# Seasandwpy/viso

Measured on AMD Instinct MI355X. Metric: stereo frames/sec at 1242x375 grey, 1/2/4/8 GPUs; pose RMSE vs reference, higher is better.
Workload: dtype f64

## Files before the change

### viso_amd/csrc/direct.hip

```cpp
#include <algorithm>
#include <cstring>

#include "device_math.hpp"
#include "direct_solve.hpp"
#include "kernels.hpp"

#ifdef VISO_PROBE
constexpr int kPRing = 4096;
constexpr int kPSt = 16;
__device__ unsigned long long g_plog[kPRing][kPSt];
__device__ unsigned long long g_pexit[kPRing];
constexpr int kPRingB = 512;
__device__ unsigned long long g_pblk[kPRingB][256][4];
__device__ unsigned long long g_pwave[kPRingB][256][16];
#ifdef VISO_PROBE_PT
constexpr int kPtRing = 128, kPtBlocks = 32, kPtStamps = 5;
__device__ unsigned long long g_ppt[kPtRing][kPtBlocks][16][kPtStamps];
#define PPT(k)                                                                                       \
    do {                                                                                             \
        if (blockIdx.x < kPtBlocks && (threadIdx.x & 63) == 0)                                       \
            g_ppt[a.probe_seq & (kPtRing - 1)][blockIdx.x][threadIdx.x >> 6][(k)] =                  \
                __builtin_amdgcn_s_memrealtime();                                                    \
    } while (0)
#endif
// ... 220 lines not shown
}

#ifdef VISO_PROBE
#ifdef VISO_PROBE_PFB
#define PFB_ADD(k) atomicAdd(&g_pfb[(k)], 1ull)
#else
#define PFB_ADD(k) ((void)0)
#endif
__device__ unsigned long long g_pfb[8];
#endif

__device__ inline double sample_cw(const uint8_t* __restrict__ img, int w, int h, double x,
                                   double y, const uint8_t* win, const CurWin& c) {
    const bool finite = (x > -1e9 && x < 1e9 && y > -1e9 && y < 1e9);
    if (__builtin_expect(finite && c.on, 1)) {
        const int ix = (int)x, iy = (int)y;
        if (__builtin_expect(ix >= c.x0 && ix + 1 < c.x0 + kCW && iy >= c.y0 && iy + 1 < c.y0 + kCW, 1)) {
            const int o = (iy - c.y0) * kCW + (ix - c.x0);
            const double d0 = (double)ld_lds_u8(win, o), d1 = (double)ld_lds_u8(win, o + 1);
            const double d2 = (double)ld_lds_u8(win, o + kCW), d3 = (double)ld_lds_u8(win, o + kCW + 1);
            const double xx = x - floor(x);
            const double yy = y - floor(y);
            return double((1 - xx) * (1 - yy) * d0 + xx * (1 - yy) * d1 + (1 - xx) * yy * d2 +
                          xx * yy * d3);
        }
        if (iy == h - 1 && ix >= c.x0 && ix + 1 < c.x0 + kCW && iy >= c.y0 && iy < c.y0 + kCW) {
            const int o = (iy - c.y0) * kCW + (ix - c.x0);
            const double d0 = (double)ld_lds_u8(win, o), d1 = (double)ld_lds_u8(win, o + 1);
            const double d2 = 0.0, d3 = 0.0;
            const double xx = x - floor(x);
            const double yy = y - floor(y);
            return double((1 - xx) * (1 - yy) * d0 + xx * (1 - yy) * d1 + (1 - xx) * yy * d2 +
                          xx * yy * d3);
        }
    }
#ifdef VISO_PROBE
    PFB_ADD(w >= 1000 ? 0 : w >= 500 ? 1 : w >= 250 ? 2 : 3);
#endif
    return sample_px(img, w, h, x, y);
}

__device__ inline double point_quotients(const Intrinsics& K, const double* pose, const double* P, double scale,
                                         double* Q, double* qt) {
    const int lane = threadIdx.x & 63;
    double Pc[3];
    mat3_vec(pose, P, Pc);
    const double x = Pc[0] + pose[9], y = Pc[1] + pose[10], z = Pc[2] + pose[11];
    const double fx = K.fx * scale, fy = K.fy * scale;
    const double zz = z * z, xy = x * y;
    const double fxx = fx * x, fyy = fy * y;
    double c1, c2, den;
    if (qt) {
        if (lane == 0) {
            double2* t2 = reinterpret_cast<double2*>(qt);
            t2[0] = make_double2(x, y);
            t2[1] = make_double2(fx, -fx);
            t2[2] = make_double2(fxx, fy);
            t2[3] = make_double2(-fy, fyy);
            t2[4] = make_double2(1.0, xy);
            t2[5] = make_double2(z, zz);
        }
        __builtin_amdgcn_fence(__ATOMIC_RELEASE, "wavefront");
        __builtin_amdgcn_wave_barrier();
        __builtin_amdgcn_fence(__ATOMIC_ACQUIRE, "wavefront");
        constexpr unsigned long long kC1 = 0x557653433210ULL, kC2 = 0x091181090888ULL,
                                     kDen = 0xABBBAABBBAAAULL;
        const int l = lane < 12 ? lane : 11;
        c1 = qt[(kC1 >> (4 * l)) & 15];
        c2 = qt[(kC2 >> (4 * l)) & 15];
        den = qt[(kDen >> (4 * l)) & 15];
    } else {
        c1 = fy;
        c1 = lane == 0 ? x : c1;
        c1 = lane == 1 ? y : c1;
        c1 = lane == 2 ? fx : c1;
        c1 = (lane == 3 || lane == 4 || lane == 6) ? -fx : c1;
        c1 = lane == 5 ? fxx : c1;
        c1 = lane == 8 ? -fy : c1;
        c1 = lane == 9 ? fyy : c1;
        c2 = 1.0;
        c2 = (lane == 3 || lane == 5 || lane >= 11) ? x : c2;
        c2 = (lane == 4 || lane == 10) ? xy : c2;
        c2 = (lane == 6 || lane == 8 || lane == 9) ? y : c2;
        den = (lane <= 2 || lane == 6 || lane == 7 || lane >= 11) ? z : zz;
    }
    double q = (c1 * c2) / den;
    if (lane == 5) q = fx + q;
    if (lane == 9) q = -fy - q;
    Q[0] = readlane_f64(q, 0);
    Q[1] = readlane_f64(q, 1);
    return lane < 12 ? q : 0.0;
}

__device__ inline unsigned factored_sources() {
    const int k = threadIdx.x & 31;
    constexpr unsigned long long lo[4] = {0x43333ccccc222222ULL, 0x9888877777ccccccULL, 0x465436543c6543c2ULL,
                                          0x9ba98ba987ba987cULL};
    constexpr unsigned long long hi[4] = {0x26543c265544ULL, 0xcba987cbaa99ULL, 0xccccccc66565ULL,
                                          0x7777777bbabaULL};
    unsigned r = 0;
#pragma unroll
    for (int q = 0; q < 4; ++q)
        r |= (unsigned)((k < 16 ? lo[q] >> (4 * k) : hi[q] >> (4 * (k - 16))) & 15) << (8 * q);
    return r;
}

__device__ inline double reduce_scatter_6_desc(const double* v) {
    const int lane = threadIdx.x & 63;
    const bool b2 = lane & 4, b3 = lane & 8;
    double a[3];
#pragma unroll
    for (int k = 0; k < 3; ++k) {
        double ra, rb;
        permlane32_swap_f64(v[k], v[3 + k], ra, rb);
        a[k] = ra + rb;
    }
    double ra, rb;
    permlane16_swap_f64(a[0], a[2], ra, rb);
    const double c0 = ra + rb;
    permlane16_swap_f64(a[1], a[1], ra, rb);
    const double c1 = ra + rb;
    double d = dsel(b3, c1, c0) + dpp_f64<0x128>(dsel(b3, c0, c1));
    const double r4 = dpp_f64<0x114>(d), l4 = dpp_f64<0x104>(d);
    d = d + dsel(b2, r4, l4);
    d = d + dpp_f64<0x4E>(d);
    d = d + dpp_f64<0xB1>(d);
    return d;
}

__device__ inline bool direct_point_rs(const DirectArgs& a, const LevelPair& fp, int lv,
                                       const double* cur_pose,
                                       const RefSample& r, const uint8_t* win, const CurWin& cw,
                                       double* out, int* idx, unsigned src_lanes, double* qt = nullptr) {
    const int lane = threadIdx.x & 63;
    const int px = (lane >> 3) - 4, py = (lane & 7) - 4;
    const double scale = kScale[lv];
    const int w = a.g.w[lv], h = a.g.h[lv];
    PPT(0);
    double Q[2];
    const double jq = point_quotients(a.K, cur_pose, r.P, scale, Q, qt);
    PPT(1);
    const double uc = scale * (Q[0] * a.K.fx + a.K.cx);
    const double vc = scale * (Q[1] * a.K.fy + a.K.cy);
    const double hp = 4.0;
    const bool good = r.ok && inside_px(uc - hp, vc - hp, w, h) && inside_px(uc + hp, vc + hp, w, h);
    if (!good) return false;
    const uint8_t* C = fp.cur;
    const double x = uc + px, y = vc + py;
    double error, g0, g1;
    const int fu = (int)floor(uc), fv = (int)floor(vc);
    if (__builtin_expect(cw.on && fu - 6 >= cw.x0 && fu + 5 <= cw.x0 + kCW - 2 && fv - 6 >= cw.y0 &&
                             fv + 5 <= cw.y0 + kCW - 2,
                         1)) {
        const bool one_binade = (__double_as_longlong(uc - 6.0) >> 52) == (__double_as_longlong(uc + 6.0) >> 52) &&
                                (__double_as_longlong(vc - 6.0) >> 52) == (__double_as_longlong(vc + 6.0) >> 52);
        if (__builtin_expect(one_binade, 1)) {
            const double xx = uc - floor(uc), yy = vc - floor(vc);
            const double w00 = (1 - xx) * (1 - yy), w10 = xx * (1 - yy), w01 = (1 - xx) * yy, w11 = xx * yy;
            const uint8_t* wb = win + ((fv + py - 1 - cw.y0) * kCW + (fu + px - 1 - cw.x0));
            auto tap = [&](int dx, int dy) { return (double)ld_lds_u8(wb, (dy + 1) * kCW + (dx + 1)); };
            const double tm0 = tap(-1, 0), t00 = tap(0, 0), t10 = tap(1, 0), t20 = tap(2, 0);
            const double tm1 = tap(-1, 1), t01 = tap(0, 1), t11 = tap(1, 1), t21 = tap(2, 1);
            const double t0m = tap(0, -1), t1m = tap(1, -1), t02 = tap(0, 2), t12 = tap(1, 2);
            auto bil = [&](double d0, double d1, double d2, double d3) {
                return double(w00 * d0 + w10 * d1 + w01 * d2 + w11 * d3);
            };
            error = r.lval - bil(t00, t10, t01, t11);
            g0 = 0.5 * (bil(t10, t20, t11, t21) - bil(tm0, t00, tm1, t01));
            g1 = 0.5 * (bil(t01, t11, t02, t12) - bil(t0m, t1m, t00, t10));
        } else {
            auto smp = [&](double sx, double sy) {
                const int o = ((int)sy - cw.y0) * kCW + ((int)sx - cw.x0);
                const double d0 = (double)ld_lds_u8(win, o), d1 = (double)ld_lds_u8(win, o + 1);
                const double d2 = (double)ld_lds_u8(win, o + kCW), d3 = (double)ld_lds_u8(win, o + kCW + 1);
                const double sxx = sx - floor(sx);
                const double syy = sy - floor(sy);
                return double((1 - sxx) * (1 - syy) * d0 + sxx * (1 - syy) * d1 + (1 - sxx) * syy * d2 +
                              sxx * syy * d3);
            };
            error = r.lval - smp(x, y);
            g0 = 0.5 * (smp(x + 1, y) - smp(x - 1, y));
            g1 = 0.5 * (smp(x, y + 1) - smp(x, y - 1));
        }
    } else {
        error = r.lval - sample_cw(C, w, h, x, y, win, cw);
        g0 = 0.5 * (sample_cw(C, w, h, x + 1, y, win, cw) - sample_cw(C, w, h, x - 1, y, win, cw));
        g1 = 0.5 * (sample_cw(C, w, h, x, y + 1, win, cw) - sample_cw(C, w, h, x, y - 1, win, cw));
    }
    PPT(2);
    const double leaf[6] = {g0 * g0, g0 * g1, g1 * g1, error * g0, error * g1, error * error};
    const double s = reduce_scatter_6_desc(leaf);
    PPT(3);
    const unsigned sa = src_lanes;
    const double p0a = bperm_f64(jq, (int)(sa & 0xff)), p1a = bperm_f64(jq, (int)((sa >> 8) & 0xff));
    const double p0b = bperm_f64(jq, (int)((sa >> 16) & 0xff)), p1b = bperm_f64(jq, (int)(sa >> 24));
    const double S0 = readlane_f64(s, 0), S1 = readlane_f64(s, 8), S2 = readlane_f64(s, 16);
    const double S3 = readlane_f64(s, 32), S4 = readlane_f64(s, 40), S5 = readlane_f64(s, 48);
    double o;
    if (lane < 21)
        o = (S0 * (p0a * p0b) + S1 * (p0a * p1b + p1a * p0b)) + S2 * (p1a * p1b);
    else if (lane < 27)
        o = S3 * p0a + S4 * p1a;
    else
        o = S5;
    *out = o;
    *idx = lane < kSums ? lane : -1;
    PPT(4);
    return true;
}

__device__ inline float tap_f32(const uint8_t* __restrict__ img, long long n, long long i) {
    return (float)ld_u8_or0(img, n, i);
}

__device__ inline bool direct_point_fast(const DirectArgs& a, const LevelPair& fp, int lv, const double* cur_pose,
                                         const double* P, float lval, const uint8_t* win, const CurWin& cw,
                                         float* out, int* idx) {
    const int lane = threadIdx.x & 63;
    const int px = (lane >> 3) - 4, py = (lane & 7) - 4;
    const double scale = kScale[lv];
    const int w = a.g.w[lv], h = a.g.h[lv];
    double Pc[3];
    mat3_vec(cur_pose, P, Pc);
    Pc[0] = Pc[0] + cur_pose[9];
    Pc[1] = Pc[1] + cur_pose[10];
    Pc[2] = Pc[2] + cur_pose[11];
    const double uc = scale * ((Pc[0] / Pc[2]) * a.K.fx + a.K.cx);
    const double vc = scale * ((Pc[1] / Pc[2]) * a.K.fy + a.K.cy);
    const double hp = 4.0;
    if (!(inside_px(uc - hp, vc - hp, w, h) && inside_px(uc + hp, vc + hp, w, h))) return false;
    const float x = (float)Pc[0], y = (float)Pc[1], z = (float)Pc[2];
    const float fxs = (float)(a.K.fx * scale), fys = (float)(a.K.fy * scale);
    const float iz = 1.0f / z, iz2 = iz * iz;
    float Jp[12];
    Jp[0] = fxs * iz;
    Jp[1] = 0.0f;
    Jp[2] = -fxs * x * iz2;
    Jp[3] = -fxs * x * y * iz2;
    Jp[4] = fxs + fxs * x * x * iz2;
    Jp[5] = -fxs * y * iz;
    Jp[6] = 0.0f;
    Jp[7] = fys * iz;
    Jp[8] = -fys * y * iz2;
    Jp[9] = -fys - fys * y * y * iz2;
    Jp[10] = fys * x * y * iz2;
    Jp[11] = fys * x * iz;
    const double fu = floor(uc), fv = floor(vc);
    const float xx = (float)(uc - fu), yy = (float)(vc - fv);
    const int ix = (int)fu + px, iy = (int)fv + py;
    float t01, t02, t10, t11, t12, t13, t20, t21, t22, t23, t31, t32;
    if (cw.on && ix - 1 >= cw.x0 && ix + 2 < cw.x0 + kCW && iy - 1 >= cw.y0 && iy + 2 < cw.y0 + kCW) {
        const int o = (iy - cw.y0) * kCW + (ix - cw.x0);
        t01 = (float)ld_lds_u8(win, o - kCW);
        t02 = (float)ld_lds_u8(win, o - kCW + 1);
        t10 = (float)ld_lds_u8(win, o - 1);
        t11 = (float)ld_lds_u8(win, o);
        t12 = (float)ld_lds_u8(win, o + 1);
        t13 = (float)ld_lds_u8(win, o + 2);
        t20 = (float)ld_lds_u8(win, o + kCW - 1);
        t21 = (float)ld_lds_u8(win, o + kCW);
        t22 = (float)ld_lds_u8(win, o + kCW + 1);
        t23 = (float)ld_lds_u8(win, o + kCW + 2);
        t31 = (float)ld_lds_u8(win, o + 2 * kCW);
        t32 = (float)ld_lds_u8(win, o + 2 * kCW + 1);
    } else {
        const uint8_t* C = fp.cur;
        const long long n = (long long)w * h, o = (long long)iy * w + ix;
        t01 = tap_f32(C, n, o - w);
        t02 = tap_f32(C, n, o - w + 1);
        t10 = tap_f32(C, n, o - 1);
        t11 = tap_f32(C, n, o);
        t12 = tap_f32(C, n, o + 1);
        t13 = tap_f32(C, n, o + 2);
        t20 = tap_f32(C, n, o + w - 1);
        t21 = tap_f32(C, n, o + w);
        t22 = tap_f32(C, n, o + w + 1);
        t23 = tap_f32(C, n, o + w + 2);
        t31 = tap_f32(C, n, o + 2 * w);
        t32 = tap_f32(C, n, o + 2 * w + 1);
    }
    const float i0 = bilerp_f32(t11, t12, t21, t22, xx, yy);
    const bool trunc_x = ix == 0 && uc > fu, trunc_y = iy == 0 && vc > fv;
    const float left = trunc_x ? i0 : bilerp_f32(t10, t11, t20, t21, xx, yy);
    const float up = trunc_y ? i0 : bilerp_f32(t01, t02, t11, t12, xx, yy);
    const float g0 = 0.5f * (bilerp_f32(t12, t13, t22, t23, xx, yy) - left);
    const float g1 = 0.5f * (bilerp_f32(t21, t22, t31, t32, xx, yy) - up);
    const float error = lval - i0;
    float J[6];
#pragma unroll
    for (int k = 0; k < 6; ++k) J[k] = -__builtin_fmaf(g0, Jp[k], g1 * Jp[6 + k]);
    float leaf[kSums];
    int e = 0;
#pragma unroll
    for (int rr = 0; rr < 6; ++rr)
#pragma unroll
        for (int c = rr; c < 6; ++c) leaf[e++] = J[rr] * J[c];
#pragma unroll
    for (int k = 0; k < 6; ++k) leaf[21 + k] = -error * J[k];
    leaf[27] = error * error;
    *out = reduce_scatter_28_f32(leaf, idx);
    return true;
}

__device__ inline float fast_lval(uint32_t t, double ur, double vr) {
    const float xx = (float)(ur - floor(ur)), yy = (float)(vr - floor(vr));
    return bilerp_f32((float)(t & 0xff), (float)((t >> 8) & 0xff), (float)((t >> 16) & 0xff), (float)(t >> 24),
                      xx, yy);
}

struct PfLds {
    uint32_t taps[kMaxTile][64];
    _Float16 lv16[kMaxTile][64];
    uint8_t win[kMaxTile][kCWBytes];
    double P[kMaxTile][3];
    double ur[kMaxTile], vr[kMaxTile];
    int ok[kMaxTile];
    int cw[kMaxTile][3];
};

struct PfPoint {
    RefSample r;
    CurWin c;
};

__device__ inline void pf_issue(const DirectArgs& a, const LevelPair& fp, int lv, int i, const double* pred,
                                bool ref, PfPoint& q) {
    if (ref) {
        ref_issue(a, fp, lv, i, q.r);
    } else {
        q.r.P[0] = a.points[3 * i];
        q.r.P[1] = a.points[3 * i + 1];
        q.r.P[2] = a.points[3 * i + 2];
    }
    double up, vp;
    project_px(pred, a.K, q.r.P, kScale[lv], up, vp);
// ... 153 lines not shown
                    const uint32_t t = (uint32_t)r.t0 | ((uint32_t)r.t1 << 8) | ((uint32_t)r.t2 << 16) |
                                       ((uint32_t)r.t3 << 24);
                    const float lval = (LV16 && !merged) ? (float)pf.lv16[local][lane] : fast_lval(t, r.ur, r.vr);
                    ok = direct_point_fast(a, fp, lv, cur_pose, r.P, lval, pf.win[local], cw, &ff, &idx);
                }
                f = (double)ff;
            } else {
                ok = direct_point_rs(a, fp, lv, cur_pose, r, pf.win[local], cw, &f, &idx, src_lanes,
                                     s_qt ? s_qt + 12 * wave : nullptr);
            }
        }
        if (!ok) {
            if (lane < kSums) s_pts[local * kSums + lane] = 0.0;
        } else if ((!FAST || lane < 32) && idx >= 0) {
            s_pts[local * kSums + idx] = f;
        }
        good_cnt += ok ? 1 : 0;
    }
    if (lane == 0 && good_cnt) atomicAdd(s_good, good_cnt);
#ifdef VISO_PROBE
    if (threadIdx.x == 0 && blockIdx.x < 256) g_pblk[a.probe_seq & (kPRingB - 1)][blockIdx.x][2] = __builtin_amdgcn_s_memrealtime();
    if (lane == 0 && blockIdx.x < 256 && wave < 15)
        g_pwave[a.probe_seq & (kPRingB - 1)][blockIdx.x][wave] = __builtin_amdgcn_s_memrealtime();
#endif
    if (s_cnt && T <= 16) {
        const int nw = T < W ? T : W;
        if (wave >= nw) return;
        int prev = 0;
        if (lane == 0)
            prev = __hip_atomic_fetch_add(s_cnt, 1, __ATOMIC_ACQ_REL, __HIP_MEMORY_SCOPE_WORKGROUP);
        prev = __builtin_amdgcn_readfirstlane(prev);
        if (prev != nw - 1) return;
        __builtin_amdgcn_fence(__ATOMIC_ACQUIRE, "workgroup");
        if (lane < kSums) {
            double v[16];
#pragma unroll
            for (int j = 0; j < 16; ++j) v[j] = j < T ? s_pts[j * kSums + lane] : 0.0;
#pragma unroll
            for (int st = 1; st < 16; st <<= 1)
#pragma unroll
                for (int j = 0; j < 16; j += 2 * st) v[j] = v[j] + v[j + st];
            double r = v[0] + 0.0;
            r = r + 0.0;
            part[(size_t)lane * kMaxTiles + b] = r;
        }
        if (lane == 0) good[b] = __hip_atomic_load(s_good, __ATOMIC_RELAXED, __HIP_MEMORY_SCOPE_WORKGROUP);
#ifdef VISO_PROBE
        if (lane == 0 && blockIdx.x < 256)
            g_pwave[a.probe_seq & (kPRingB - 1)][blockIdx.x][15] = __builtin_amdgcn_s_memrealtime();
#endif
        return;
    }
    __syncthreads();
    for (int k = wave; k < kSums; k += W) {
        const double v = lane < T ? s_pts[lane * kSums + k] : 0.0;
        const double r = wave_tree_sum_dpp(v);
        if (lane == 0) part[(size_t)k * kMaxTiles + b] = r;
    }
    if (threadIdx.x == 0) good[b] = *s_good;
    __syncthreads();
}

__device__ inline void state_to_pose(const double* st, double* pose) {
    double q[4] = {st[0], st[1], st[2], st[3]};
    quat_to_matrix(q, pose);
    pose[9] = st[4];
    pose[10] = st[5];
    pose[11] = st[6];
}


__device__ inline void load_partials(const double* __restrict__ part, const int* __restrict__ good,
                                     int n_tiles, double* v, int& gg) {
    const int t = threadIdx.x;
    if (t < n_tiles) {
#pragma unroll
        for (int k = 0; k < kSums; ++k) v[k] = part[(size_t)k * kMaxTiles + t];
        gg = good[t];
    } else {
#pragma unroll
        for (int k = 0; k < kSums; ++k) v[k] = 0.0;
        gg = 0;
    }
}

__device__ inline void reduce_partials(const double* v, int gg, SolveLds& L) {
    const int t = threadIdx.x, wave = t >> 6, lane = t & 63;
    if (t < 256) {
        int idx;
        const double f = reduce_scatter_28(v, &idx);
        if (lane < 32 && idx >= 0) L.red[wave][idx] = f;
        const int g = wave_sum_int(gg);
        if (lane == 0) L.g[wave] = g;
    }
    __syncthreads();
    if (t < kSums) L.S[t] = (L.red[0][t] + L.red[1][t]) + (L.red[2][t] + L.red[3][t]);
    if (t == 0) L.ngood = (L.g[0] + L.g[1]) + (L.g[2] + L.g[3]);
    __syncthreads();
}

__device__ inline void lds_barrier() { asm volatile("s_waitcnt lgkmcnt(0)\n\ts_barrier" ::: "memory"); }

template <bool FAST>
__device__ void solve_continue(const DirectArgs& a, const FramePair& fpair, int lv, SolveLds& L,
                               double* stats, double* s_pose, double* s_pts, int* s_good, PfLds& pf) {
    const int t = threadIdx.x, wave = t >> 6;
    double* part = a.s.cont_part + (size_t)blockIdx.x * kMaxTiles * kSums;
    int* good = a.s.cont_good + (size_t)blockIdx.x * kMaxTiles;
    const LevelPair fp = level_pair(fpair, lv);
    for (int iter = 1; iter < 100 && L.cont; ++iter) {
        if (t == 0) state_to_pose(L.state, s_pose);
        __syncthreads();
        double pose[12];
#pragma unroll
        for (int k = 0; k < 12; ++k) pose[k] = s_pose[k];
        for (int b = 0; b < a.n_tiles; ++b) {
            if (t == 0) *s_good = 0;
            prefetch_tile(a, lv, b, pose, fpair.pose_last, true, wave, kWaves, pf, &fpair);
            __syncthreads();
            direct_tile_pf<FAST>(a, fp, lv, pose, b, pf, false, part, good, s_pts, s_good);
        }
        __threadfence_block();
        __syncthreads();
        double v[kSums];
        int gg = 0;
        if (t < 256) load_partials(part, good, a.n_tiles, v, gg);
        reduce_partials(v, gg, L);
        if (wave == 0) {
            if (FAST)
                solve_wave0_ldlt(L, iter, stats);
            else
                solve_wave0(L, iter, stats);
        }
        __syncthreads();
    }
}

__device__ inline void prefetch_point(const DirectArgs& a, int lv, int i, bool solve, int sl,
                                      RefSample& r, CurWin& cw) {
    ref_issue(a, level_pair(a.fp, lv), lv, i, r);
    double pred[12];
    if (!solve) {
        for (int k = 0; k < 12; ++k) pred[k] = a.pose_seed[k];
    } else {
        double sp[7];
        for (int k = 0; k < 7; ++k) sp[k] = a.s.state[sl * kStateStride + k];
        state_to_pose(sp, pred);
    }
    double up, vp;
    project_px(pred, a.K, r.P, kScale[lv], up, vp);
    win_issue(a.fp.cur.l[lv], a.g.w[lv], a.g.h[lv], up, vp, cw);
}

__device__ inline void after_solve(const DirectArgs& a, bool merged, SolveLds& L, double* s_last,
                                   double* s_pose) {
    if (merged) {
        state_to_pose(L.state, s_last);
        if (blockIdx.x == 0) {
            for (int k = 0; k < 7; ++k) a.s.state[kLevels * kStateStride + k] = L.state[k];
            if (a.prev_pose_out) store_frame_pose(a.prev_pose_out, s_last, a.prev_ready);
            log_pose(a.prev_log, a.prev_log_host, a.prev_log_index, s_last);
            log_frame(a.flog, a.prev_log_index, L);
        }
        double q[4];
        quat_from_matrix(s_last, q);
        for (int k = 0; k < 4; ++k) L.state[k] = q[k];
        L.state[4] = s_last[9];
        L.state[5] = s_last[10];
        L.state[6] = s_last[11];
    }
    state_to_pose(L.state, s_pose);
}

template <bool FAST>
__global__ __launch_bounds__(kThreads, 4) void direct_level_kernel(const double* __restrict__ pre_part,
                                                                 const int* __restrict__ pre_good, int pre_hdr,
                                                                 DirectArgs a) {
    PROBE_DECL();
    __builtin_amdgcn_s_setprio(1);
    __shared__ SolveLds L;
    __shared__ double s_pose[12];
    __shared__ double s_last[12];
    __shared__ double s_pts[kMaxTile * kSums];
    __shared__ int s_good;
    __shared__ int s_cnt;
    __shared__ int s_arrive;
    __shared__ PfLds s_pf;
#ifndef VISO_NO_QT
    __shared__ __attribute__((aligned(16))) double s_qt[FAST ? 2 : kWaves * 12];
    double* const qt = FAST ? nullptr : s_qt;
#else
    double* const qt = nullptr;
#endif
    const int lv = a.level;
    const bool merged = a.merged && lv == kLevels - 1;
    const int prev = lv + 1;
    const bool solve = prev < kLevels || merged;
    const int sl = merged ? 0 : prev;
    const int t = threadIdx.x, wave = t >> 6, lane = t & 63;
    const bool tiles = lv >= 0 && (int)blockIdx.x < a.n_tiles;
    double v[kSums];
    int gg = 0;
    if (((pre_hdr >> 16) & 1) && t < 256) load_partials(pre_part, pre_good, pre_hdr & 0xffff, v, gg);
    const bool pf_wave = !solve || (wave & 3) != 0;
    double st[7];
    if (t == 256 || (solve && tiles && pf_wave)) {
        if (!solve) {
            quat_from_matrix(a.pose_seed, st);
            st[4] = a.pose_seed[9];
            st[5] = a.pose_seed[10];
            st[6] = a.pose_seed[11];
        } else {
#pragma unroll
            for (int k = 0; k < 7; ++k) st[k] = a.s.state[sl * kStateStride + k];
        }
    }
    if (t == 0) {
        s_arrive = 0;
        s_good = 0;
        s_cnt = 0;
#ifdef VISO_PROBE
        for (int k = 0; k < kPSt; ++k) pst[k] = 0;
        pst[0] = probe_t0;
        if (blockIdx.x < 256) g_pblk[a.probe_seq & (kPRingB - 1)][blockIdx.x][0] = probe_t0;
#endif
    }
    lds_barrier();

    if (t == 256) {
        for (int k = 0; k < 7; ++k) {
            L.state[k] = st[k];
            L.best[k] = st[k];
        }
        L.cost = 0.0;
        L.last_cost = 0.0;
        L.cont = 0;
        asm volatile("s_waitcnt lgkmcnt(0)" ::: "memory");
        atomicAdd(&s_arrive, 1);
    }
    if (solve && t < 256) {
        int idx;
        const double f = reduce_scatter_28(v, &idx);
        if (lane < 32 && idx >= 0) L.red[wave][idx] = f;
        const int g = wave_sum_int(gg);
        if (lane == 0) L.g[wave] = g;
        asm volatile("s_waitcnt lgkmcnt(0)" ::: "memory");
        if (lane == 0) atomicAdd(&s_arrive, 1);
    }
    if (wave == 0) PST(1);

    const bool solver = solve && wave == 0;
    if (tiles && pf_wave) {
        double pred[12];
        if (!solve) {
            for (int k = 0; k < 12; ++k) pred[k] = a.pose_seed[k];
        } else {
            state_to_pose(st, pred);
        }
        const int first = solve ? wave - (wave >> 2) - 1 : wave;
        const int stride = solve ? kWaves - kWaves / 4 : kWaves;
        prefetch_tile(a, lv, blockIdx.x, pred, merged ? pred : a.fp.pose_last, true, first, stride, s_pf);
#ifdef VISO_PROBE
        asm volatile("s_waitcnt vmcnt(0) lgkmcnt(0)" ::: "memory");
        if (blockIdx.x == 0 && lane == 0) atomicMax(&pst[9], __builtin_amdgcn_s_memrealtime());
#endif
    }

    if (solver) {
        __builtin_amdgcn_s_setprio(3);
        while (__hip_atomic_load(&s_arrive, __ATOMIC_RELAXED, __HIP_MEMORY_SCOPE_WORKGROUP) < 5)
            __builtin_amdgcn_s_sleep(1);
        if (lane < kSums) L.S[lane] = (L.red[0][lane] + L.red[1][lane]) + (L.red[2][lane] + L.red[3][lane]);
        if (lane == 0) L.ngood = (L.g[0] + L.g[1]) + (L.g[2] + L.g[3]);
        PST(2);
        double* stp = (a.stats && blockIdx.x == 0) ? a.stats + (size_t)kStats * sl : nullptr;
#ifdef VISO_PROBE
        unsigned long long stamps[5] = {probe_t0, probe_t0, probe_t0, probe_t0, probe_t0};
        if (FAST)
            solve_wave0_ldlt(L, 0, stp, stamps);
        else
            solve_wave0(L, 0, stp, stamps);
        if (blockIdx.x == 0 && lane == 0)
            for (int k = 0; k < 4; ++k) pst[3 + k] = stamps[k];
        if (blockIdx.x == 0 && lane == 0) pst[12] = stamps[4];
#else
        if (FAST)
            solve_wave0_ldlt(L, 0, stp);
        else
            solve_wave0(L, 0, stp);
#endif
        PST(7);
        __builtin_amdgcn_s_setprio(1);
    }
    if (!solve && wave == 0 && lane == 0) {
        while (__hip_atomic_load(&s_arrive, __ATOMIC_RELAXED, __HIP_MEMORY_SCOPE_WORKGROUP) < 1)
            __builtin_amdgcn_s_sleep(1);
    }
    if (wave == 0 && lane == 0 && !L.cont) after_solve(a, merged, L, s_last, s_pose);
    const unsigned src_lanes = FAST ? 0u : factored_sources();
    __syncthreads();
    if (__builtin_expect(solve && L.cont, 0)) {
        double* stp = (a.stats && blockIdx.x == 0) ? a.stats + (size_t)kStats * sl : nullptr;
        solve_continue<FAST>(a, merged ? a.prev : a.fp, sl, L, stp, s_pose, s_pts, &s_good, s_pf);
        if (t == 0) {
            after_solve(a, merged, L, s_last, s_pose);
            s_good = 0;
        }
        __syncthreads();
        if (tiles) {
            double pose[12];
#pragma unroll
            for (int k = 0; k < 12; ++k) pose[k] = s_pose[k];
            prefetch_tile(a, lv, blockIdx.x, pose, merged ? s_last : a.fp.pose_last, true, wave, kWaves, s_pf);
        }
        __syncthreads();
    }
    if (wave == 0) PST(8);
#ifdef VISO_PROBE
    if (t == 0 && blockIdx.x < 256) g_pblk[a.probe_seq & (kPRingB - 1)][blockIdx.x][1] = __builtin_amdgcn_s_memrealtime();
#endif
    const int out = lv >= 0 ? lv : kLevels;
    if (blockIdx.x == 0 && t == 0 && !merged) {
        for (int k = 0; k < 7; ++k) a.s.state[out * kStateStride + k] = L.state[k];
        if (lv < 0 && a.pose_out) {
            store_frame_pose(a.pose_out, s_pose, a.ready);
            log_pose(a.log, a.log_host, a.log_index, s_pose);
            log_frame(a.flog, a.log_index, L);
        }
    }
    if (blockIdx.x == 0 && t == 0 && merged)
        for (int k = 0; k < 7; ++k) a.s.state[lv * kStateStride + k] = L.state[k];
    if (tiles) {
        LevelPair fp = level_pair(a.fp, lv);
        if (merged) fp.pose_last = s_last;
        double pose[12];
#pragma unroll
        for (int k = 0; k < 12; ++k) pose[k] = s_pose[k];
        direct_tile_pf<FAST>(a, fp, lv, pose, blockIdx.x, s_pf, merged, a.s.part + (size_t)lv * kMaxTiles * kSums,
                       a.s.good + lv * kMaxTiles, s_pts, &s_good, &s_cnt, qt, src_lanes);
    }
#ifdef VISO_PROBE
    __syncthreads();
    const unsigned long long t_exit = __builtin_amdgcn_s_memrealtime();
    const int slot = a.probe_seq & (kPRing - 1);
    if (t == 0 && blockIdx.x < 256) g_pblk[a.probe_seq & (kPRingB - 1)][blockIdx.x][3] = t_exit;
    if (blockIdx.x == 0 && t == 0) {
        pst[11] = t_exit;
        pst[15] = (unsigned long long)(lv + 1) | ((unsigned long long)merged << 8) |
                  ((unsigned long long)a.n_tiles << 16);
        for (int k = 0; k < kPSt; ++k) g_plog[slot][k] = pst[k];
    }
#endif
}

constexpr int kRigTiles = kMaxTiles;

__device__ __host__ inline int rig_reduce_waves(int n_tiles) { return n_tiles <= 64 ? 1 : n_tiles <= 128 ? 2 : 4; }

struct RigCamArgs {
    DirectArgs d;
    const double* Ad;
    double E[12];
};

struct RigArgs {
    RigCamArgs cam[kMaxRigCams];
    int n_cams;
    int tile_off[kMaxRigCams + 1];
    int level;
    double* state;
    const double* seed;
    double* stats;
    double* pose_out;
    double* log;
    int log_index;
    double* cam_last;
    int merged;
    double* prev_pose_out;
    double* prev_log;
    int prev_log_index;
};

__device__ inline void rig_compose(const double* E, const double* T, double* out) {
#pragma unroll
    for (int i = 0; i < 3; ++i) {
#pragma unroll
        for (int j = 0; j < 3; ++j)
            out[3 * i + j] = (E[3 * i] * T[j] + E[3 * i + 1] * T[3 + j]) + E[3 * i + 2] * T[6 + j];
        out[9 + i] = ((E[3 * i] * T[9] + E[3 * i + 1] * T[10]) + E[3 * i + 2] * T[11]) + E[9 + i];
    }
}

__device__ inline int rig_camera(const RigArgs& ra, int b) {
    int c = 0;
#pragma unroll
    for (int k = 1; k < kMaxRigCams; ++k) {
        const int off = ra.tile_off[k];
        if (k < ra.n_cams && b >= off) c = k;
    }
    return c;
}

__device__ inline void rig_contrib(int q, double (*red)[kSums], const double* Ad, double* sM, double* con) {
    const int lane = threadIdx.x & 63;
    if (q > 1 && lane < kSums) {
        const double v = q == 2 ? red[0][lane] + red[1][lane]
                                : (red[0][lane] + red[1][lane]) + (red[2][lane] + red[3][lane]);
        red[0][lane] = v;
    }
    asm volatile("s_waitcnt lgkmcnt(0)" ::: "memory");
    const double* S = red[0];
    if (lane < 36) {
        const int i = lane / 6, j = lane - 6 * (lane / 6);
        double m = 0.0;
#pragma unroll
        for (int k = 0; k < 6; ++k) {
            const int a = i < k ? i : k, bb = i < k ? k : i;
            const double h = S[a * 6 - (a * (a - 1)) / 2 + (bb - a)];
            m = k == 0 ? h * Ad[j] : m + h * Ad[6 * k + j];
        }
        sM[lane] = m;
    }
    asm volatile("s_waitcnt lgkmcnt(0)" ::: "memory");
    int ei = 0, ej = 0;
    {
        int e = lane < 21 ? lane : 0, r = 0;
        while (e >= 6 - r) {
            e -= 6 - r;
            ++r;
        }
        ei = r;
        ej = r + e;
    }
    double v = 0.0;
    if (lane < 21) {
#pragma unroll
        for (int k = 0; k < 6; ++k) v = k == 0 ? Ad[ei] * sM[ej] : v + Ad[6 * k + ei] * sM[6 * k + ej];
    } else if (lane < 27) {
        const int i = lane - 21;
#pragma unroll
        for (int k = 0; k < 6; ++k) v = k == 0 ? Ad[i] * S[21] : v + Ad[6 * k + i] * S[21 + k];
    } else if (lane == 27) {
        v = S[27];
    }
    if (lane < kSums) con[lane] = v;
    asm volatile("s_waitcnt lgkmcnt(0)" ::: "memory");
}

__device__ inline void rig_fold(const RigArgs& ra, const double (*con)[kSums], const int (*g)[4], SolveLds& L) {
    const int lane = threadIdx.x & 63;
    int ng = 0;
    for (int c = 0; c < ra.n_cams; ++c) {
        const int q = rig_reduce_waves(ra.cam[c].d.n_tiles);
        for (int j = 0; j < q; ++j) ng += g[c][j];
    }
    if (lane < kSums) {
        double acc = con[0][lane];
        for (int c = 1; c < ra.n_cams; ++c) acc = acc + con[c][lane];
        L.S[lane] = acc;
    }
    if (lane == 0) L.ngood = ng;
    asm volatile("s_waitcnt lgkmcnt(0)" ::: "memory");
}

constexpr size_t kRigPartBytes = (size_t)kLevels * kRigTiles * kSums * 8;
constexpr size_t kRigScratchBytes = kRigPartBytes + (size_t)kLevels * kRigTiles * 4;

template <bool FAST, bool MERGED>
__global__ __launch_bounds__(kRigThreads) void rig_level_kernel(const char* __restrict__ pre_scratch,
                                                                const double* __restrict__ pre_ad, int pre_hdr,
                                                                int pre_t01, int pre_t23, RigArgs ra) {
    __shared__ SolveLds L;
    __shared__ double s_red[kMaxRigCams][4][kSums];
    __shared__ int s_g[kMaxRigCams][4];
    __shared__ double s_M[kMaxRigCams][36];
    __shared__ double s_Ad[kMaxRigCams][36];
    __shared__ double s_con[kMaxRigCams][kSums];
    __shared__ int s_camarr[kMaxRigCams];
    __shared__ double s_pose[12];
    __shared__ double s_last[12];
    __shared__ double s_pts[kMaxTile * kSums];
    __shared__ int s_good;
    __shared__ int s_cnt;
    __shared__ int s_arrive;
// ... 569 lines not shown
```

### viso_amd/csrc/direct_solve.hpp

```cpp
#pragma once

#include "common.hpp"
#include "device_math.hpp"


namespace viso {

constexpr int kSolveSums = 28;
constexpr int kSolveStateStride = 8;

struct SolveLds {
    double red[4][kSolveSums];
    double S[kSolveSums];
    int g[4];
    int ngood;
    double state[kSolveStateStride], best[kSolveStateStride];
    double cost, last_cost;
    int cont;
};

#define SPROBE(k)                                                   \
    do {                                                            \
        if (stamps) stamps[(k)] = __builtin_amdgcn_s_memrealtime(); \
    } while (0)

__device__ __attribute__((always_inline)) inline void solve_finish(SolveLds& L, const double* update, double h, int iter, double* stats,
                                    unsigned long long* stamps) {
    const int lane = threadIdx.x & 63;
    const bool in = lane < 36;
    const int ngood = L.ngood;
    double cost = L.cost + L.S[27];
    cost /= ngood;
    const double lastCost = L.last_cost;
    const bool nan_update = isnan(update[0]);
    const bool cost_up = iter > 0 && cost > lastCost;
    const bool converged = (1 - cost / (double)lastCost) < 0.005;
    SE3d T21;
#pragma unroll
    for (int k = 0; k < 4; ++k) T21.q[k] = L.state[k];
#pragma unroll
    for (int k = 0; k < 3; ++k) T21.t[k] = L.state[4 + k];
    SE3d E;
    {
        const double eps = 1e-10;
        const double* w = update + 3;
        const double theta_sq = (w[0] * w[0] + w[1] * w[1]) + w[2] * w[2];
        const double theta = sqrt(theta_sq);
        const double half_theta = 0.5 * theta;
        double sn, cs;
        sincos((lane & 1) ? theta : half_theta, &sn, &cs);
        const double s_half = readlane_f64(sn, 0), c_half = readlane_f64(cs, 0);
        const double s_th = readlane_f64(sn, 1), c_th = readlane_f64(cs, 1);
        double imag, real;
        if (theta < eps) {
            const double theta_po4 = theta_sq * theta_sq;
            imag = 0.5 - (1.0 / 48.0) * theta_sq + (1.0 / 3840.0) * theta_po4;
            real = 1.0 - 0.5 * theta_sq + (1.0 / 384.0) * theta_po4;
        } else {
            imag = s_half / theta;
            real = c_half;
        }
        E.q[0] = imag * w[0];
        E.q[1] = imag * w[1];
        E.q[2] = imag * w[2];
        E.q[3] = real;
        double V[9];
        if (theta < eps) {
            quat_to_matrix(E.q, V);
        } else {
            const double O[9] = {0.0, -w[2], w[1], w[2], 0.0, -w[0], -w[1], w[0], 0.0};
            double O2[9];
#pragma unroll
            for (int i = 0; i < 3; ++i)
#pragma unroll
                for (int j = 0; j < 3; ++j)
                    O2[3 * i + j] = (O[3 * i + 0] * O[0 + j] + O[3 * i + 1] * O[3 + j]) + O[3 * i + 2] * O[6 + j];
            const double th2 = theta * theta;
            const double c1 = (1.0 - c_th) / th2;
            const double c2 = (theta - s_th) / (th2 * theta);
#pragma unroll
            for (int i = 0; i < 9; ++i) {
                const double id = (i % 4 == 0) ? 1.0 : 0.0;
                V[i] = (id + c1 * O[i]) + c2 * O2[i];
            }
        }
        mat3_vec(V, update, E.t);
    }
    SPROBE(3);
    T21 = se3_mul(E, T21);
    if (stats) {
        if (in) stats[2 + lane] = h;
        if (lane == 0) {
            stats[0] = ngood;
            stats[1] = cost;
            for (int k = 0; k < 6; ++k) stats[38 + k] = L.S[21 + k];
            for (int k = 0; k < 6; ++k) stats[44 + k] = update[k];
        }
    }
    if (lane == 0) {
        int cont = 1;
        if (nan_update) {
            for (int k = 0; k < 7; ++k) L.state[k] = L.best[k];
            cont = 0;
        } else {
            for (int k = 0; k < 4; ++k) L.state[k] = T21.q[k];
            for (int k = 0; k < 3; ++k) L.state[4 + k] = T21.t[k];
            if (cost_up) {
                for (int k = 0; k < 7; ++k) L.state[k] = L.best[k];
                cont = 0;
            } else if (converged) {
                cont = 0;
            } else {
                for (int k = 0; k < 7; ++k) L.best[k] = L.state[k];
                L.last_cost = cost;
            }
        }
        L.cost = cost;
        L.cont = cont;
    }
}



__device__ __attribute__((always_inline)) inline void solve_after_lu(SolveLds& L, const double* A, const int* tr,
                                                                      double h, int iter, double* stats,
                                                                      unsigned long long* stamps);

__device__ __attribute__((always_inline)) inline void solve_wave0_rep(SolveLds& L, int iter, double* stats,
                                   unsigned long long* stamps = nullptr) {
    const int lane = threadIdx.x & 63;
    const int row = lane / 6, col = lane - 6 * (lane / 6);
    const bool in = lane < 36;
    const int r0 = row < col ? row : col, c0 = row < col ? col : row;
    const double h = in ? L.S[r0 * 6 - (r0 * (r0 - 1)) / 2 + (c0 - r0)] : 0.0;
    double A[36];
    int tr[6];
#ifdef VISO_LU_TWICE
#pragma clang loop unroll(disable)
    for (int rep = 0; rep < 2; ++rep) {
#endif
#pragma unroll
    for (int r = 0; r < 6; ++r)
#pragma unroll
        for (int c = 0; c < 6; ++c) {
            const int r1 = r < c ? r : c, c1 = r < c ? c : r;
            A[6 * r + c] = L.S[r1 * 6 - (r1 * (r1 - 1)) / 2 + (c1 - r1)];
        }
#pragma unroll
    for (int k = 0; k < 6; ++k) {
        int p = k;
        double best = fabs(A[7 * k]);
#pragma unroll
        for (int i = k + 1; i < 6; ++i) {
            const double s = fabs(A[6 * i + k]);
            if (s > best) {
                best = s;
                p = i;
            }
        }
        p = __builtin_amdgcn_readfirstlane(p);
        tr[k] = p;
        if (__builtin_amdgcn_readfirstlane(best != 0.0 ? 1 : 0)) {
#pragma unroll
            for (int i = k + 1; i < 6; ++i) {
                if (p == i) {
#pragma unroll
                    for (int c = 0; c < 6; ++c) {
                        const double tmp = A[6 * k + c];
                        A[6 * k + c] = A[6 * i + c];
                        A[6 * i + c] = tmp;
                    }
                }
            }
            const double piv = A[7 * k];
#pragma unroll
            for (int i = k + 1; i < 6; ++i) A[6 * i + k] = A[6 * i + k] / piv;
        }
#pragma unroll
        for (int i = k + 1; i < 6; ++i)
#pragma unroll
            for (int c = k + 1; c < 6; ++c) A[6 * i + c] = A[6 * i + c] - A[6 * i + k] * A[6 * k + c];
    }
#ifdef VISO_LU_TWICE
    if (rep == 0) {
        asm volatile("" ::"v"(A[35]), "v"(A[0]));
        if (stamps) stamps[4] = __builtin_amdgcn_s_memrealtime();
    }
    }
#endif
    SPROBE(0);
    solve_after_lu(L, A, tr, h, iter, stats, stamps);
}

__device__ __attribute__((always_inline)) inline void solve_after_lu(SolveLds& L, const double* A, const int* tr,
                                                                      double h, int iter, double* stats,
                                                                      unsigned long long* stamps) {
    const int lane = threadIdx.x & 63;
    const int cc = lane < 6 ? lane : 0;
    int pos = cc;
#pragma unroll
    for (int k = 0; k < 6; ++k) {
        if (pos == k) pos = tr[k];
        else if (pos == tr[k]) pos = k;
    }
    double x[6];
#pragma unroll
    for (int r = 0; r < 6; ++r) x[r] = (r == pos) ? 1.0 : 0.0;
#pragma unroll
    for (int j = 0; j < 6; ++j)
#pragma unroll
        for (int i = j + 1; i < 6; ++i) x[i] = x[i] - A[6 * i + j] * x[j];
#pragma unroll
    for (int j = 5; j >= 0; --j) {
        x[j] = x[j] / A[7 * j];
#pragma unroll
        for (int i = 0; i < j; ++i) x[i] = x[i] - A[6 * i + j] * x[j];
    }
    SPROBE(1);
    double update[6];
    {
        double* Tt = &L.red[0][0];
        if (lane < 6) {
#pragma unroll
            for (int r = 0; r < 6; ++r) Tt[6 * r + lane] = x[r];
        }
        asm volatile("s_waitcnt lgkmcnt(0)" ::: "memory");
        double s = 0.0;
        if (lane < 6) {
            const double* row = Tt + 6 * lane;
            s = row[0] * L.S[21];
#pragma unroll
            for (int c = 1; c < 6; ++c) s = s + row[c] * L.S[21 + c];
        }
#pragma unroll
        for (int r = 0; r < 6; ++r) update[r] = readlane_f64(s, r);
    }
    SPROBE(2);
    solve_finish(L, update, h, iter, stats, stamps);
}


__device__ inline double bperm_f64(double v, int src) {
    const long long b = __double_as_longlong(v);
    const int lo = __builtin_amdgcn_ds_bpermute(src * 4, (int)(b & 0xffffffffLL));
    const int hi = __builtin_amdgcn_ds_bpermute(src * 4, (int)(b >> 32));
    return __longlong_as_double(((long long)hi << 32) | (unsigned int)lo);
}

__device__ __attribute__((always_inline)) inline void solve_wave0_lane(SolveLds& L, int iter, double* stats,
                                                                        unsigned long long* stamps = nullptr) {
    const int lane = threadIdx.x & 63;
    const int r = lane / 6, c = lane - 6 * (lane / 6);
    const bool in = lane < 36;
    const int r0 = r < c ? r : c, c0 = r < c ? c : r;
    const double h = in ? L.S[r0 * 6 - (r0 * (r0 - 1)) / 2 + (c0 - r0)] : 0.0;
    double a = h;
    int tr[6];
#pragma unroll
    for (int k = 0; k < 6; ++k) {
        int p = k;
        double best = fabs(readlane_f64(a, 7 * k));
#pragma unroll
        for (int i = k + 1; i < 6; ++i) {
            const double s = fabs(readlane_f64(a, 6 * i + k));
            if (s > best) {
                best = s;
                p = i;
            }
        }
        p = __builtin_amdgcn_readfirstlane(p);
        tr[k] = p;
        if (__builtin_amdgcn_readfirstlane(best != 0.0 ? 1 : 0)) {
            if (p != k) a = bperm_f64(a, r == k ? 6 * p + c : (r == p ? 6 * k + c : lane));
            const double piv = readlane_f64(a, 7 * k);
            if (in && r > k && c == k) a = a / piv;
        }
        if (k < 5) {
            const double lk = bperm_f64(a, 6 * r + k), kc = bperm_f64(a, 6 * k + c);
            if (in && r > k && c > k) a = a - lk * kc;
        }
    }
    double* T = &L.red[0][0];
    if (in) T[lane] = a;
    asm volatile("s_waitcnt lgkmcnt(0)" ::: "memory");
    double A[36];
#pragma unroll
    for (int i = 0; i < 36; ++i) A[i] = T[i];
    asm volatile("s_waitcnt lgkmcnt(0)" ::: "memory");
    SPROBE(0);
    solve_after_lu(L, A, tr, h, iter, stats, stamps);
}


__device__ __attribute__((always_inline)) inline void solve_wave0(SolveLds& L, int iter, double* stats,
                                                                   unsigned long long* stamps = nullptr) {
#ifdef VISO_SOLVE_LANE
    solve_wave0_lane(L, iter, stats, stamps);
#else
    solve_wave0_rep(L, iter, stats, stamps);
#endif
}

__device__ __attribute__((always_inline)) inline void solve_wave0_ldlt(SolveLds& L, int iter, double* stats,
                                        unsigned long long* stamps = nullptr) {
    const int lane = threadIdx.x & 63;
    const int row = lane / 6, col = lane - 6 * (lane / 6);
    const bool in = lane < 36;
    const int r0 = row < col ? row : col, c0 = row < col ? col : row;
    const double h = in ? L.S[r0 * 6 - (r0 * (r0 - 1)) / 2 + (c0 - r0)] : 0.0;
    double A[21];
#pragma unroll
    for (int i = 0; i < 6; ++i)
#pragma unroll
        for (int j = 0; j <= i; ++j) A[i * (i + 1) / 2 + j] = L.S[j * 6 - (j * (j - 1)) / 2 + (i - j)];
    double b[6];
#pragma unroll
    for (int k = 0; k < 6; ++k) b[k] = L.S[21 + k];
    double Dinv[6];
    bool bad = false;
#pragma unroll
    for (int k = 0; k < 6; ++k) {
        double d = A[k * (k + 1) / 2 + k];
#pragma unroll
        for (int j = 0; j < k; ++j) {
            const double lkj = A[k * (k + 1) / 2 + j];
            d = __builtin_fma(-lkj * lkj, A[j * (j + 1) / 2 + j], d);
        }
        bad = bad || !(d > 0.0) || !(d < 1e300);
        const double di = 1.0 / d;
        Dinv[k] = di;
        A[k * (k + 1) / 2 + k] = d;
#pragma unroll
        for (int i = k + 1; i < 6; ++i) {
            double s = A[i * (i + 1) / 2 + k];
#pragma unroll
            for (int j = 0; j < k; ++j)
                s = __builtin_fma(-A[i * (i + 1) / 2 + j] * A[j * (j + 1) / 2 + j], A[k * (k + 1) / 2 + j], s);
            A[i * (i + 1) / 2 + k] = s * di;
        }
    }
    SPROBE(0);
    double y[6];
#pragma unroll
    for (int i = 0; i < 6; ++i) {
        double s = b[i];
#pragma unroll
        for (int j = 0; j < i; ++j) s = __builtin_fma(-A[i * (i + 1) / 2 + j], y[j], s);
        y[i] = s;
    }
    double update[6];
#pragma unroll
    for (int i = 5; i >= 0; --i) {
        double s = y[i] * Dinv[i];
#pragma unroll
        for (int j = i + 1; j < 6; ++j) s = __builtin_fma(-A[j * (j + 1) / 2 + i], update[j], s);
        update[i] = s;
    }
    if (bad)
#pragma unroll
        for (int k = 0; k < 6; ++k) update[k] = __builtin_nan("");
    SPROBE(1);
    SPROBE(2);
    solve_finish(L, update, h, iter, stats, stamps);
}

}
```

Baseline: 20260.

## Carry solver state in registers and defer merged-frame global writes

The solver's final state is now passed back in registers through a SolveOut struct, so the critical path no longer re-reads LDS. The merged-frame global stores and logging (state, pose output, logs) move out of after_solve to a later point after the barrier, shortening the serial lane-0 section before __syncthreads. The sampler's fast stencil path is widened: when the sample point does not share one binade, a wave-wide __all check still allows the 12-tap LDS stencil, using per-sample bilinear weights. This adds a wave vote and some extra floating-point work on that rare path, and changes the quaternion seeding logic.

```diff
diff --git a/viso_amd/csrc/direct.hip b/viso_amd/csrc/direct.hip
--- a/viso_amd/csrc/direct.hip
+++ b/viso_amd/csrc/direct.hip
@@ -396,22 +396,40 @@
     if (__builtin_expect(cw.on && fu - 6 >= cw.x0 && fu + 5 <= cw.x0 + kCW - 2 && fv - 6 >= cw.y0 &&
                              fv + 5 <= cw.y0 + kCW - 2,
                          1)) {
-        const bool one_binade = (__double_as_longlong(uc - 6.0) >> 52) == (__double_as_longlong(uc + 6.0) >> 52) &&
-                                (__double_as_longlong(vc - 6.0) >> 52) == (__double_as_longlong(vc + 6.0) >> 52);
-        if (__builtin_expect(one_binade, 1)) {
-            const double xx = uc - floor(uc), yy = vc - floor(vc);
-            const double w00 = (1 - xx) * (1 - yy), w10 = xx * (1 - yy), w01 = (1 - xx) * yy, w11 = xx * yy;
+        const bool share = (uc + 6.0) - 6.0 == uc && (vc + 6.0) - 6.0 == vc;
+        bool stencil = share;
+        const double xp = x + 1, xm = x - 1, yp = y + 1, ym = y - 1;
+        if (__builtin_expect(!share, 0)) {
+            const int bx = fu + px, by = fv + py;
+            stencil = __all((int)x == bx && (int)xp == bx + 1 && (int)xm == bx - 1 && (int)y == by &&
+                            (int)yp == by + 1 && (int)ym == by - 1);
+        }
+        if (__builtin_expect(stencil, 1)) {
             const uint8_t* wb = win + ((fv + py - 1 - cw.y0) * kCW + (fu + px - 1 - cw.x0));
             auto tap = [&](int dx, int dy) { return (double)ld_lds_u8(wb, (dy + 1) * kCW + (dx + 1)); };
             const double tm0 = tap(-1, 0), t00 = tap(0, 0), t10 = tap(1, 0), t20 = tap(2, 0);
             const double tm1 = tap(-1, 1), t01 = tap(0, 1), t11 = tap(1, 1), t21 = tap(2, 1);
             const double t0m = tap(0, -1), t1m = tap(1, -1), t02 = tap(0, 2), t12 = tap(1, 2);
-            auto bil = [&](double d0, double d1, double d2, double d3) {
-                return double(w00 * d0 + w10 * d1 + w01 * d2 + w11 * d3);
-            };
-            error = r.lval - bil(t00, t10, t01, t11);
-            g0 = 0.5 * (bil(t10, t20, t11, t21) - bil(tm0, t00, tm1, t01));
-            g1 = 0.5 * (bil(t01, t11, t02, t12) - bil(t0m, t1m, t00, t10));
+            if (__builtin_expect(share, 1)) {
+                const double xx = uc - floor(uc), yy = vc - floor(vc);
+                const double w00 = (1 - xx) * (1 - yy), w10 = xx * (1 - yy), w01 = (1 - xx) * yy, w11 = xx * yy;
+                auto bil = [&](double d0, double d1, double d2, double d3) {
+                    return double(w00 * d0 + w10 * d1 + w01 * d2 + w11 * d3);
+                };
+                error = r.lval - bil(t00, t10, t01, t11);
+                g0 = 0.5 * (bil(t10, t20, t11, t21) - bil(tm0, t00, tm1, t01));
+                g1 = 0.5 * (bil(t01, t11, t02, t12) - bil(t0m, t1m, t00, t10));
+            } else {
+                auto bil = [&](double sx, double sy, double d0, double d1, double d2, double d3) {
+                    const double sxx = sx - floor(sx);
+                    const double syy = sy - floor(sy);
+                    return double((1 - sxx) * (1 - syy) * d0 + sxx * (1 - syy) * d1 + (1 - sxx) * syy * d2 +
+                                  sxx * syy * d3);
+                };
+                error = r.lval - bil(x, y, t00, t10, t01, t11);
+                g0 = 0.5 * (bil(xp, y, t10, t20, t11, t21) - bil(xm, y, tm0, t00, tm1, t01));
+                g1 = 0.5 * (bil(x, yp, t01, t11, t02, t12) - bil(x, ym, t0m, t1m, t00, t10));
+            }
         } else {
             auto smp = [&](double sx, double sy) {
                 const int o = ((int)sy - cw.y0) * kCW + ((int)sx - cw.x0);
@@ -423,8 +441,8 @@
                               sxx * syy * d3);
             };
             error = r.lval - smp(x, y);
-            g0 = 0.5 * (smp(x + 1, y) - smp(x - 1, y));
-            g1 = 0.5 * (smp(x, y + 1) - smp(x, y - 1));
+            g0 = 0.5 * (smp(xp, y) - smp(xm, y));
+            g1 = 0.5 * (smp(x, yp) - smp(x, ym));
         }
     } else {
         error = r.lval - sample_cw(C, w, h, x, y, win, cw);
@@ -884,24 +902,36 @@
     win_issue(a.fp.cur.l[lv], a.g.w[lv], a.g.h[lv], up, vp, cw);
 }
 
-__device__ inline void after_solve(const DirectArgs& a, bool merged, SolveLds& L, double* s_last,
+__device__ inline void after_solve(bool merged, const double* st, SolveLds& L, double* s_last, double* s_prev,
                                    double* s_pose) {
+    double pose[12];
     if (merged) {
-        state_to_pose(L.state, s_last);
-        if (blockIdx.x == 0) {
-            for (int k = 0; k < 7; ++k) a.s.state[kLevels * kStateStride + k] = L.state[k];
-            if (a.prev_pose_out) store_frame_pose(a.prev_pose_out, s_last, a.prev_ready);
-            log_pose(a.prev_log, a.prev_log_host, a.prev_log_index, s_last);
-            log_frame(a.flog, a.prev_log_index, L);
-        }
-        double q[4];
-        quat_from_matrix(s_last, q);
-        for (int k = 0; k < 4; ++k) L.state[k] = q[k];
-        L.state[4] = s_last[9];
-        L.state[5] = s_last[10];
-        L.state[6] = s_last[11];
-    }
-    state_to_pose(L.state, s_pose);
+        double last[12];
+        state_to_pose(st, last);
+        for (int k = 0; k < 12; ++k) s_last[k] = last[k];
+        for (int k = 0; k < 7; ++k) s_prev[k] = st[k];
+        double seed[7];
+        if ((last[0] + last[4]) + last[8] > 0.0)
+            quat_from_matrix(last, seed);
+        else
+            quat_from_matrix(s_last, seed);
+        seed[4] = last[9];
+        seed[5] = last[10];
+        seed[6] = last[11];
+        state_to_pose(seed, pose);
+        for (int k = 0; k < 7; ++k) L.state[k] = seed[k];
+    } else {
+        state_to_pose(st, pose);
+    }
+    for (int k = 0; k < 12; ++k) s_pose[k] = pose[k];
+}
+
+__device__ inline void merged_outputs(const DirectArgs& a, const SolveLds& L, const double* s_last,
+                                      const double* s_prev) {
+    for (int k = 0; k < 7; ++k) a.s.state[kLevels * kStateStride + k] = s_prev[k];
+    if (a.prev_pose_out) store_frame_pose(a.prev_pose_out, s_last, a.prev_ready);
+    log_pose(a.prev_log, a.prev_log_host, a.prev_log_index, s_last);
+    log_frame(a.flog, a.prev_log_index, L);
 }
 
 template <bool FAST>
@@ -913,6 +943,7 @@
     __shared__ SolveLds L;
     __shared__ double s_pose[12];
     __shared__ double s_last[12];
+    __shared__ double s_prev[kStateStride];
     __shared__ double s_pts[kMaxTile * kSums];
     __shared__ int s_good;
     __shared__ int s_cnt;
@@ -998,6 +1029,8 @@
 #endif
     }
 
+    SolveOut fin;
+    fin.cont = 0;
     if (solver) {
         __builtin_amdgcn_s_setprio(3);
         while (__hip_atomic_load(&s_arrive, __ATOMIC_RELAXED, __HIP_MEMORY_SCOPE_WORKGROUP) < 5)
@@ -1009,17 +1042,17 @@
 #ifdef VISO_PROBE
         unsigned long long stamps[5] = {probe_t0, probe_t0, probe_t0, probe_t0, probe_t0};
         if (FAST)
-            solve_wave0_ldlt(L, 0, stp, stamps);
+            solve_wave0_ldlt(L, 0, stp, stamps, &fin);
         else
-            solve_wave0(L, 0, stp, stamps);
+            solve_wave0(L, 0, stp, stamps, &fin);
         if (blockIdx.x == 0 && lane == 0)
             for (int k = 0; k < 4; ++k) pst[3 + k] = stamps[k];
         if (blockIdx.x == 0 && lane == 0) pst[12] = stamps[4];
 #else
         if (FAST)
-            solve_wave0_ldlt(L, 0, stp);
+            solve_wave0_ldlt(L, 0, stp, nullptr, &fin);
         else
-            solve_wave0(L, 0, stp);
+            solve_wave0(L, 0, stp, nullptr, &fin);
 #endif
         PST(7);
         __builtin_amdgcn_s_setprio(1);
@@ -1027,15 +1060,17 @@
     if (!solve && wave == 0 && lane == 0) {
         while (__hip_atomic_load(&s_arrive, __ATOMIC_RELAXED, __HIP_MEMORY_SCOPE_WORKGROUP) < 1)
             __builtin_amdgcn_s_sleep(1);
-    }
-    if (wave == 0 && lane == 0 && !L.cont) after_solve(a, merged, L, s_last, s_pose);
+        for (int k = 0; k < 7; ++k) fin.state[k] = L.state[k];
+    }
+    if (wave == 0 && lane == 0 && !fin.cont) after_solve(merged, fin.state, L, s_last, s_prev, s_pose);
     const unsigned src_lanes = FAST ? 0u : factored_sources();
     __syncthreads();
     if (__builtin_expect(solve && L.cont, 0)) {
         double* stp = (a.stats && blockIdx.x == 0) ? a.stats + (size_t)kStats * sl : nullptr;
         solve_continue<FAST>(a, merged ? a.prev : a.fp, sl, L, stp, s_pose, s_pts, &s_good, s_pf);
         if (t == 0) {
-            after_solve(a, merged, L, s_last, s_pose);
+            for (int k = 0; k < 7; ++k) fin.state[k] = L.state[k];
+            after_solve(merged, fin.state, L, s_last, s_prev, s_pose);
             s_good = 0;
         }
         __syncthreads();
@@ -1060,8 +1095,10 @@
             log_frame(a.flog, a.log_index, L);
         }
     }
-    if (blockIdx.x == 0 && t == 0 && merged)
+    if (blockIdx.x == 0 && t == 0 && merged) {
+        merged_outputs(a, L, s_last, s_prev);
         for (int k = 0; k < 7; ++k) a.s.state[lv * kStateStride + k] = L.state[k];
+    }
     if (tiles) {
         LevelPair fp = level_pair(a.fp, lv);
         if (merged) fp.pose_last = s_last;
diff --git a/viso_amd/csrc/direct_solve.hpp b/viso_amd/csrc/direct_solve.hpp
--- a/viso_amd/csrc/direct_solve.hpp
+++ b/viso_amd/csrc/direct_solve.hpp
@@ -19,13 +19,18 @@
     int cont;
 };
 
+struct SolveOut {
+    double state[7];
+    int cont;
+};
+
 #define SPROBE(k)                                                   \
     do {                                                            \
         if (stamps) stamps[(k)] = __builtin_amdgcn_s_memrealtime(); \
     } while (0)
 
 __device__ __attribute__((always_inline)) inline void solve_finish(SolveLds& L, const double* update, double h, int iter, double* stats,
-                                    unsigned long long* stamps) {
+                                    unsigned long long* stamps, SolveOut* fin) {
     const int lane = threadIdx.x & 63;
     const bool in = lane < 36;
     const int ngood = L.ngood;
@@ -98,22 +103,21 @@
         }
     }
     if (lane == 0) {
-        int cont = 1;
-        if (nan_update) {
-            for (int k = 0; k < 7; ++k) L.state[k] = L.best[k];
-            cont = 0;
-        } else {
-            for (int k = 0; k < 4; ++k) L.state[k] = T21.q[k];
-            for (int k = 0; k < 3; ++k) L.state[4 + k] = T21.t[k];
-            if (cost_up) {
-                for (int k = 0; k < 7; ++k) L.state[k] = L.best[k];
-                cont = 0;
-            } else if (converged) {
-                cont = 0;
-            } else {
-                for (int k = 0; k < 7; ++k) L.best[k] = L.state[k];
-                L.last_cost = cost;
-            }
+        double ns[7];
+        for (int k = 0; k < 4; ++k) ns[k] = T21.q[k];
+        for (int k = 0; k < 3; ++k) ns[4 + k] = T21.t[k];
+        const bool revert = nan_update || cost_up;
+        if (revert)
+            for (int k = 0; k < 7; ++k) ns[k] = L.best[k];
+        for (int k = 0; k < 7; ++k) L.state[k] = ns[k];
+        const int cont = !revert && !converged;
+        if (cont) {
+            for (int k = 0; k < 7; ++k) L.best[k] = ns[k];
+            L.last_cost = cost;
+        }
+        if (fin) {
+            for (int k = 0; k < 7; ++k) fin->state[k] = ns[k];
+            fin->cont = cont;
         }
         L.cost = cost;
         L.cont = cont;
@@ -124,10 +128,10 @@
 
 __device__ __attribute__((always_inline)) inline void solve_after_lu(SolveLds& L, const double* A, const int* tr,
                                                                       double h, int iter, double* stats,
-                                                                      unsigned long long* stamps);
+                                                                      unsigned long long* stamps, SolveOut* fin);
 
 __device__ __attribute__((always_inline)) inline void solve_wave0_rep(SolveLds& L, int iter, double* stats,
-                                   unsigned long long* stamps = nullptr) {
+                                   unsigned long long* stamps = nullptr, SolveOut* fin = nullptr) {
     const int lane = threadIdx.x & 63;
     const int row = lane / 6, col = lane - 6 * (lane / 6);
     const bool in = lane < 36;
@@ -189,12 +193,12 @@
     }
 #endif
     SPROBE(0);
-    solve_after_lu(L, A, tr, h, iter, stats, stamps);
+    solve_after_lu(L, A, tr, h, iter, stats, stamps, fin);
 }
 
 __device__ __attribute__((always_inline)) inline void solve_after_lu(SolveLds& L, const double* A, const int* tr,
                                                                       double h, int iter, double* stats,
-                                                                      unsigned long long* stamps) {
+                                                                      unsigned long long* stamps, SolveOut* fin) {
     const int lane = threadIdx.x & 63;
     const int cc = lane < 6 ? lane : 0;
     int pos = cc;
@@ -236,7 +240,7 @@
         for (int r = 0; r < 6; ++r) update[r] = readlane_f64(s, r);
     }
     SPROBE(2);
-    solve_finish(L, update, h, iter, stats, stamps);
+    solve_finish(L, update, h, iter, stats, stamps, fin);
 }
 
 
@@ -248,7 +252,7 @@
 }
 
 __device__ __attribute__((always_inline)) inline void solve_wave0_lane(SolveLds& L, int iter, double* stats,
-                                                                        unsigned long long* stamps = nullptr) {
+                                                                        unsigned long long* stamps = nullptr, SolveOut* fin = nullptr) {
     const int lane = threadIdx.x & 63;
     const int r = lane / 6, c = lane - 6 * (lane / 6);
     const bool in = lane < 36;
@@ -288,21 +292,21 @@
     for (int i = 0; i < 36; ++i) A[i] = T[i];
     asm volatile("s_waitcnt lgkmcnt(0)" ::: "memory");
     SPROBE(0);
-    solve_after_lu(L, A, tr, h, iter, stats, stamps);
+    solve_after_lu(L, A, tr, h, iter, stats, stamps, fin);
 }
 
 
 __device__ __attribute__((always_inline)) inline void solve_wave0(SolveLds& L, int iter, double* stats,
-                                                                   unsigned long long* stamps = nullptr) {
+                                                                   unsigned long long* stamps = nullptr, SolveOut* fin = nullptr) {
 #ifdef VISO_SOLVE_LANE
-    solve_wave0_lane(L, iter, stats, stamps);
+    solve_wave0_lane(L, iter, stats, stamps, fin);
 #else
-    solve_wave0_rep(L, iter, stats, stamps);
+    solve_wave0_rep(L, iter, stats, stamps, fin);
 #endif
 }
 
 __device__ __attribute__((always_inline)) inline void solve_wave0_ldlt(SolveLds& L, int iter, double* stats,
-                                        unsigned long long* stamps = nullptr) {
+                                        unsigned long long* stamps = nullptr, SolveOut* fin = nullptr) {
     const int lane = threadIdx.x & 63;
     const int row = lane / 6, col = lane - 6 * (lane / 6);
     const bool in = lane < 36;
@@ -361,7 +365,7 @@
         for (int k = 0; k < 6; ++k) update[k] = __builtin_nan("");
     SPROBE(1);
     SPROBE(2);
-    solve_finish(L, update, h, iter, stats, stamps);
-}
-
-}
+    solve_finish(L, update, h, iter, stats, stamps, fin);
+}
+
+}
```

New measurement: 20460, median of 6. No clear change (+1.0%).
